# wolfecameron/GIST

Hardware: AMD Instinct MI355X
Metric: epochs/sec (higher is better)
Workload: dtype f32 (projection products from 3 bf16 pieces per operand = all 24 bits, 6 cross terms, fp32 accumulation)

## Files before the change

### gist_amd/csrc/gemm_b3.hip

```cpp
#include <stdlib.h>
#include <string.h>

#include <type_traits>

#include "common.h"

namespace gist {

typedef __bf16 bf16x8 __attribute__((ext_vector_type(8)));
typedef float b3_f32x4 __attribute__((ext_vector_type(4)));

constexpr int B3_TM = 256, B3_TN = 128, B3_BK = 32;
constexpr int B3_THREADS = 512;
constexpr int B3_STAGES = 2;
constexpr int B3_SKEW = 16;
constexpr int B3_KT_BYTES = B3_BK * 6;
constexpr int B3_A_BYTES = B3_TM * B3_KT_BYTES;
constexpr int B3_B_BYTES = B3_TN * B3_KT_BYTES;
constexpr int B3_BUF_BYTES = B3_A_BYTES + B3_B_BYTES;

__device__ __forceinline__ uint32_t b3_pack(__bf16 lo, __bf16 hi) {
    return (uint32_t)__builtin_bit_cast(unsigned short, lo) |
           ((uint32_t)__builtin_bit_cast(unsigned short, hi) << 16);
}

__device__ __forceinline__ void b3_emit(const float (&v)[8], uint16_t *__restrict__ dst) {
    uint32_t w[3][4];
#pragma unroll
    for (int j = 0; j < 4; ++j) {
        __bf16 p[2][3];
#pragma unroll
        for (int h = 0; h < 2; ++h) {
            const float x = v[2 * j + h];
            p[h][0] = (__bf16)x;
            const float r1 = x - (float)p[h][0];
            p[h][1] = (__bf16)r1;
            const float r2 = r1 - (float)p[h][1];
            p[h][2] = (__bf16)r2;
        }
#pragma unroll
        for (int q = 0; q < 3; ++q) w[q][j] = b3_pack(p[0][q], p[1][q]);
    }
#pragma unroll
    for (int q = 0; q < 3; ++q)
        *reinterpret_cast<uint4 *>(dst + 8 * q) = make_uint4(w[q][0], w[q][1], w[q][2], w[q][3]);
}

__global__ __launch_bounds__(256) void b3_dual_split_kernel(B3Dual d, int64_t ldd_r, int64_t ldd_t,
                                                            float keep) {
    __shared__ float tile[64][65];
    const int c0 = blockIdx.x * 64, r0 = blockIdx.y * 64;
    const int t = threadIdx.x;
    const int c4 = (t & 15) * 4;
    const uint64_t sm = d.seed * 0x9E3779B97F4A7C15ULL;
    const float inv24 = 1.0f / 16777216.0f;
#pragma unroll
    for (int i = 0; i < 4; ++i) {
        const int rr = (t >> 4) + 16 * i;
        const int64_t r = r0 + rr;
        float v[4] = {0.f, 0.f, 0.f, 0.f};
        if (r < d.rows) {
            const float *p = d.src + r * d.ld + c0 + c4;
            if (c0 + c4 + 3 < d.cols && d.vec4) {
                const float4 q = *reinterpret_cast<const float4 *>(p);
                v[0] = q.x; v[1] = q.y; v[2] = q.z; v[3] = q.w;
            } else {
#pragma unroll
                for (int j = 0; j < 4; ++j)
                    if (c0 + c4 + j < d.cols) v[j] = p[j];
            }
            if (d.p > 0.f) {
                const uint64_t idx0 = d.offset + (uint64_t)r * (uint64_t)d.cols + (uint64_t)(c0 + c4);
#pragma unroll
                for (int j = 0; j < 4; ++j) {
                    const uint64_t idx = idx0 + j;
                    const uint64_t h = splitmix64((idx >> 1) + sm);
                    const uint32_t w = (idx & 1) ? (uint32_t)(h >> 32) : (uint32_t)h;
                    v[j] *= ((float)(w >> 8) * inv24 >= d.p) ? keep : 0.f;
                }
            }
        }
        tile[rr][c4 + 0] = v[0]; tile[rr][c4 + 1] = v[1];
        tile[rr][c4 + 2] = v[2]; tile[rr][c4 + 3] = v[3];
    }
    __syncthreads();
    if (d.col_partials != nullptr && t < 64 && c0 + t < d.cols && r0 < d.rows) {
        float s0 = 0.f, s1 = 0.f, s2 = 0.f, s3 = 0.f;
#pragma unroll
        for (int r = 0; r < 64; r += 4) {
            s0 += tile[r][t]; s1 += tile[r + 1][t]; s2 += tile[r + 2][t]; s3 += tile[r + 3][t];
        }
        d.col_partials[(int64_t)blockIdx.y * d.cols + c0 + t] = (s0 + s1) + (s2 + s3);
    }
    const int kb = t & 7;
#pragma unroll
    for (int i = 0; i < 2; ++i) {
        const int q = (t >> 3) + 32 * i;
        if (d.dst_r != nullptr && r0 + q < d.rows && c0 + kb * 8 < ldd_r) {
            float v[8];
#pragma unroll
            for (int j = 0; j < 8; ++j) v[j] = tile[q][kb * 8 + j];
            b3_emit(v, d.dst_r + ((int64_t)(r0 + q) * ldd_r + c0 + kb * 8) * 3);
        }
        if (d.dst_t != nullptr && c0 + q < d.cols && r0 + kb * 8 < ldd_t) {
            float v[8];
#pragma unroll
            for (int j = 0; j < 8; ++j) v[j] = tile[kb * 8 + j][q];
            b3_emit(v, d.dst_t + ((int64_t)(c0 + q) * ldd_t + r0 + kb * 8) * 3);
        }
    }
}

struct B3Args {
    const uint16_t *a; int64_t lda;
    const uint16_t *b; int64_t ldb;
    const float *bias;
    float *c; int64_t ldc;
    int m, n, kpad;
    int tiles_m, tiles_n;
    int kt_per_split;
    int64_t split_stride;
    int dp_tiles, tail_splits, tail_kt;
    float *tail_partials;
};

template <int NI>
__device__ __forceinline__ void b3_dma_offsets(int64_t ld, int rows, int row0, int first, int lane,
                                                uint32_t (&off)[NI]) {
#pragma unroll
    for (int jj = 0; jj < NI; ++jj) {
        const int inst = first + jj;
        const int slot = (inst % 3) * 64 + lane;
        const int rs = slot / 12;
        const int chunk = (slot % 12) ^ ((rs >> 3) << 1);
        const int r = (inst / 3) * 16 + rs;
        const int dr = min(r, rows - 1 - row0);
        off[jj] = (uint32_t)((int64_t)dr * ld * 6 + chunk * 16);
    }
}

__device__ __forceinline__ void b3_mfma(b3_f32x4 &acc, const bf16x8 &a, const bf16x8 &b) {
    asm volatile("v_mfma_f32_16x16x32_bf16 %0, %1, %2, %0" : "+v"(acc) : "v"(a), "v"(b));
}

template <int NI>
__device__ __forceinline__ void b3_dma_image(const char *base, const uint32_t (&off)[NI], char *image,
                                             int first) {
    __amdgpu_buffer_rsrc_t rsrc = __builtin_amdgcn_make_buffer_rsrc(
        const_cast<char *>(base), 0, 0x7fffffff, 0x00020000);
#pragma unroll
    for (int jj = 0; jj < NI; ++jj)
        __builtin_amdgcn_raw_ptr_buffer_load_lds(
            rsrc, (__attribute__((address_space(3))) void *)(image + (first + jj) * 1024), 16, off[jj],
            0, 0, 0);
}

__global__ __launch_bounds__(B3_THREADS, 2) void gemm_b3_kernel(B3Args g) {
    extern __shared__ __attribute__((aligned(16))) char b3_smem[];
    constexpr int NI = 4, NJ = 4;
    const int nwg = g.dp_tiles;
    const int orig = blockIdx.x;
    const bool tail = orig >= nwg;
    const int tail_tile = tail ? (orig - nwg) / g.tail_splits : 0;
    const int tail_slice = tail ? (orig - nwg) % g.tail_splits : 0;
    const int qd = nwg / kXcds, rm = nwg % kXcds, xcd = orig % kXcds;
    const int L = tail ? nwg + tail_tile
                       : (xcd < rm ? xcd * (qd + 1) : rm * (qd + 1) + (xcd - rm) * qd) + orig / kXcds;
    constexpr int GM = 8;
    const int width = GM * g.tiles_n;
    const int group = L / width;
    const int first_m = group * GM;
    const int gsz = min(g.tiles_m - first_m, GM);
    const int bm = first_m + (L % width) % gsz;
    const int bn = (L % width) / gsz;
    const int row0 = bm * B3_TM, col0 = bn * B3_TN;
    const int kt0 = tail ? tail_slice * g.tail_kt : (int)blockIdx.y * g.kt_per_split;
    const int n_kt = min(g.kpad / B3_BK - kt0, tail ? g.tail_kt : g.kt_per_split);

    const int lane = threadIdx.x & 63;
    const int wave = __builtin_amdgcn_readfirstlane(threadIdx.x >> 6);
    const int wm = wave >> 1, wn = wave & 1;
    const int rr = lane & 15, kg = lane >> 4;

    b3_f32x4 acc[NI][NJ];
#pragma unroll
    for (int i = 0; i < NI; ++i)
#pragma unroll
        for (int j = 0; j < NJ; ++j)
#pragma unroll
            for (int e = 0; e < 4; ++e) acc[i][j][e] = 0.f;

    constexpr int NWAVES = B3_THREADS / 64;
    constexpr int DA = B3_TM / 16 * 3 / NWAVES, DB = B3_TN / 16 * 3 / NWAVES;
    uint32_t offA[DA], offB[DB];
    b3_dma_offsets<DA>(g.lda, g.m, row0, DA * wave, lane, offA);
    b3_dma_offsets<DB>(g.ldb, g.n, col0, DB * wave, lane, offB);
    const char *originA = reinterpret_cast<const char *>(g.a) + (int64_t)row0 * g.lda * 6 + (int64_t)kt0 * B3_KT_BYTES;
    const char *originB = reinterpret_cast<const char *>(g.b) + (int64_t)col0 * g.ldb * 6 + (int64_t)kt0 * B3_KT_BYTES;
    auto dma = [&](int buf, int kt) {
        char *sa = b3_smem + buf * B3_BUF_BYTES;
        b3_dma_image<DA>(originA + (int64_t)kt * B3_KT_BYTES, offA, sa, DA * wave);
        b3_dma_image<DB>(originB + (int64_t)kt * B3_KT_BYTES, offB, sa + B3_A_BYTES, DB * wave);
    };

    const char *fa[B3_STAGES][3], *fb[B3_STAGES][3];
#pragma unroll
    for (int p = 0; p < 3; ++p) {
        const int c = 3 * kg + p;
        const int in_slab = (rr * 12 + (c ^ ((rr >> 3) << 1))) * 16;
#pragma unroll
        for (int st = 0; st < B3_STAGES; ++st) {
            fa[st][p] = b3_smem + st * B3_BUF_BYTES + wm * NI * 3072 + in_slab;
            fb[st][p] = b3_smem + st * B3_BUF_BYTES + B3_A_BYTES + wn * NJ * 3072 + in_slab;
        }
    }

    const bool live = __builtin_amdgcn_readfirstlane(row0 + wm * (16 * NI) < g.m);
    bf16x8 a[NI][3], b[NJ][3];
    auto read_head = [&](auto st_c) {
        constexpr int st = decltype(st_c)::value;
        if (!live) return;
#pragma unroll
        for (int j = 0; j < NJ; ++j) b[j][0] = *reinterpret_cast<const bf16x8 *>(fb[st][0] + j * 3072);
#pragma unroll
        for (int i = 0; i < NI; ++i) a[i][1] = *reinterpret_cast<const bf16x8 *>(fa[st][1] + i * 3072);
#pragma unroll
        for (int i = 0; i < NI; ++i) a[i][2] = *reinterpret_cast<const bf16x8 *>(fa[st][2] + i * 3072);
    };
    auto read_rest = [&](auto st_c) {
        constexpr int st = decltype(st_c)::value;
        if (!live) return;
#pragma unroll
        for (int j = 0; j < NJ; ++j) b[j][1] = *reinterpret_cast<const bf16x8 *>(fb[st][1] + j * 3072);
#pragma unroll
        for (int i = 0; i < NI; ++i) a[i][0] = *reinterpret_cast<const bf16x8 *>(fa[st][0] + i * 3072);
#pragma unroll
        for (int j = 0; j < NJ; ++j) b[j][2] = *reinterpret_cast<const bf16x8 *>(fb[st][2] + j * 3072);
    };
    constexpr int pa[6] = {1, 2, 1, 0, 0, 0};
    constexpr int pb[6] = {0, 0, 1, 0, 1, 2};
    constexpr int B3_MID = 4 * NI * NJ;

    dma(0, 0);
    __builtin_amdgcn_s_waitcnt(0x0f70);
    __syncthreads();
    dma(1, 1);
    read_head(std::integral_constant<int, 0>{});

    auto mfmas = [&](auto t0_c, auto t1_c) {
        constexpr int t0 = decltype(t0_c)::value, t1 = decltype(t1_c)::value;
        if (!live) return;
#pragma unroll
        for (int t = t0; t < t1; ++t) {
            const int term = t / (NI * NJ), i = (t % (NI * NJ)) / NJ, j = t % NJ;
            b3_mfma(acc[i][j], a[i][pa[term]], b[j][pb[term]]);
        }
    };
    const int last_kt = n_kt - 1;
    auto kstep = [&](auto cur_c, auto late_c, int kt) {
        constexpr int cur = decltype(cur_c)::value;
        constexpr int skew = decltype(late_c)::value * B3_SKEW;
        using I = std::integral_constant<int, 0>;
        __builtin_amdgcn_sched_barrier(0);
        __builtin_amdgcn_s_setprio(1);
        mfmas(I{}, std::integral_constant<int, skew>{});
        __builtin_amdgcn_sched_barrier(0);
        read_rest(cur_c);
        __builtin_amdgcn_sched_barrier(0);
        mfmas(std::integral_constant<int, skew>{}, std::integral_constant<int, B3_MID>{});
        __builtin_amdgcn_sched_barrier(0);
        __builtin_amdgcn_s_waitcnt(0x0070);
        __syncthreads();
        mfmas(std::integral_constant<int, B3_MID>{}, std::integral_constant<int, B3_MID + skew>{});
        __builtin_amdgcn_sched_barrier(0);
        dma(cur, min(kt + 2, last_kt));
        read_head(std::integral_constant<int, cur ^ 1>{});
        __builtin_amdgcn_sched_barrier(0);
        mfmas(std::integral_constant<int, B3_MID + skew>{}, std::integral_constant<int, 6 * NI * NJ>{});
        __builtin_amdgcn_s_setprio(0);
        __builtin_amdgcn_sched_barrier(0);
    };
    auto run = [&](auto late_c) {
        using C0 = std::integral_constant<int, 0>;
        using C1 = std::integral_constant<int, 1>;
        for (int kt = 0; kt < n_kt; kt += 2) {
            kstep(C0{}, late_c, kt);
            kstep(C1{}, late_c, kt + 1);
        }
    };
    if (wave >= 4) run(std::integral_constant<int, 1>{});
    else run(std::integral_constant<int, 0>{});
    __builtin_amdgcn_s_waitcnt(0x0070);

    asm volatile("s_nop 15\n\ts_nop 15" ::: "memory");
    const int rows_valid = min(g.m - row0, B3_TM);
    if (tail) {
        const bool rows_live = wm * (16 * NI) < rows_valid;
        b3_f32x4 *mine = reinterpret_cast<b3_f32x4 *>(g.tail_partials) +
                         (int64_t)(tail_tile * g.tail_splits + tail_slice) * (NI * NJ * B3_THREADS) + threadIdx.x;
        if (rows_live) {
#pragma unroll
            for (int i = 0; i < NI; ++i)
#pragma unroll
                for (int j = 0; j < NJ; ++j) mine[(i * NJ + j) * B3_THREADS] = acc[i][j];
        }
        return;
    }
    float *cbase = g.c + (int64_t)blockIdx.y * g.split_stride + (int64_t)row0 * g.ldc + col0;
    __amdgpu_buffer_rsrc_t crsrc = __builtin_amdgcn_make_buffer_rsrc(
        cbase, 0, (int)((int64_t)rows_valid * g.ldc * 4), 0x00020000);
    const uint32_t ldc_b = (uint32_t)g.ldc * 4;
    uint32_t cvoff[NJ];
    float bv[NJ];
#pragma unroll
    for (int j = 0; j < NJ; ++j) {
        const int cl = wn * (16 * NJ) + j * 16 + rr;
        const bool ok = col0 + cl < g.n;
        cvoff[j] = ok ? (uint32_t)(wm * (16 * NI) + 4 * kg) * ldc_b + (uint32_t)cl * 4 : 0x7fffffffu;
        bv[j] = (g.bias != nullptr && ok) ? g.bias[col0 + cl] : 0.f;
    }
#pragma unroll
    for (int i = 0; i < NI; ++i)
#pragma unroll
        for (int e = 0; e < 4; ++e) {
            const uint32_t roff = (uint32_t)(i * 16 + e) * ldc_b;
#pragma unroll
            for (int j = 0; j < NJ; ++j) {
                const float v = acc[i][j][e] + bv[j];
                if (rows_valid == B3_TM)
                    __builtin_amdgcn_raw_buffer_store_b32(__float_as_uint(v), crsrc, cvoff[j], roff, 0);
                else
                    __builtin_amdgcn_raw_buffer_store_b32(__float_as_uint(v), crsrc, cvoff[j] + roff, 0, 0);
            }
        }
}

constexpr int B3W_TN = 256;
constexpr int B3W_B_BYTES = B3W_TN * B3_KT_BYTES;
constexpr int B3W_LDS_BYTES = B3_A_BYTES + 2 * B3W_B_BYTES;

__global__ __launch_bounds__(B3_THREADS, 1) void gemm_b3_wide_kernel(B3Args g) {
    extern __shared__ __attribute__((aligned(16))) char b3_smem[];
    constexpr int NI = 4, NJ = 8;
    const int nwg = g.dp_tiles;
    const int orig = blockIdx.x;
    const int qd = nwg / kXcds, rm = nwg % kXcds, xcd = orig % kXcds;
    const int L = (xcd < rm ? xcd * (qd + 1) : rm * (qd + 1) + (xcd - rm) * qd) + orig / kXcds;
    constexpr int GM = 8;
    const int width = GM * g.tiles_n;
    const int group = L / width;
    const int first_m = group * GM;
    const int gsz = min(g.tiles_m - first_m, GM);
    const int bm = first_m + (L % width) % gsz;
    const int bn = (L % width) / gsz;
    const int row0 = bm * B3_TM, col0 = bn * B3W_TN;
    const int n_kt = g.kpad / B3_BK;

    const int lane = threadIdx.x & 63;
    const int wave = __builtin_amdgcn_readfirstlane(threadIdx.x >> 6);
    const int wm = wave >> 1, wn = wave & 1;
    const int rr = lane & 15, kg = lane >> 4;

    b3_f32x4 acc[NI][NJ];
#pragma unroll
    for (int i = 0; i < NI; ++i)
#pragma unroll
        for (int j = 0; j < NJ; ++j)
#pragma unroll
            for (int e = 0; e < 4; ++e) acc[i][j][e] = 0.f;

    constexpr int NWAVES = B3_THREADS / 64;
    constexpr int DA = B3_TM / 16 * 3 / NWAVES, DB = B3W_TN / 16 * 3 / NWAVES;
    uint32_t offA[DA], offB[DB];
    b3_dma_offsets<DA>(g.lda, g.m, row0, DA * wave, lane, offA);
    b3_dma_offsets<DB>(g.ldb, g.n, col0, DB * wave, lane, offB);
    const char *originA = reinterpret_cast<const char *>(g.a) + (int64_t)row0 * g.lda * 6;
    const char *originB = reinterpret_cast<const char *>(g.b) + (int64_t)col0 * g.ldb * 6;
    auto dma = [&](int bbuf, int kt) {
        b3_dma_image<DA>(originA + (int64_t)kt * B3_KT_BYTES, offA, b3_smem, DA * wave);
        b3_dma_image<DB>(originB + (int64_t)kt * B3_KT_BYTES, offB, b3_smem + B3_A_BYTES + bbuf * B3W_B_BYTES,
                         DB * wave);
    };

    const char *fa[3], *fb[2][3];
#pragma unroll
    for (int p = 0; p < 3; ++p) {
        const int c = 3 * kg + p;
        const int in_slab = (rr * 12 + (c ^ ((rr >> 3) << 1))) * 16;
        fa[p] = b3_smem + wm * NI * 3072 + in_slab;
#pragma unroll
        for (int st = 0; st < 2; ++st) fb[st][p] = b3_smem + B3_A_BYTES + st * B3W_B_BYTES + wn * NJ * 3072 + in_slab;
    }

    auto body = [&](auto live_c) {
        constexpr bool live = decltype(live_c)::value;
        bf16x8 a[NI][3], b[2][3];
        auto read_a = [&](auto p_c) {
            constexpr int p = decltype(p_c)::value;
            if constexpr (!live) return;
#pragma unroll
            for (int i = 0; i < NI; ++i) a[i][p] = *reinterpret_cast<const bf16x8 *>(fa[p] + i * 3072);
        };
        auto read_b = [&](auto st_c, auto pair_c, auto p_c) {
            constexpr int st = decltype(st_c)::value, pair = decltype(pair_c)::value, p = decltype(p_c)::value;
            if constexpr (!live) return;
#pragma unroll
            for (int jj = 0; jj < 2; ++jj) b[jj][p] = *reinterpret_cast<const bf16x8 *>(fb[st][p] + (2 * pair + jj) * 3072);
        };
        constexpr int pa[6] = {1, 2, 1, 0, 0, 0};
        constexpr int pb[6] = {0, 0, 1, 0, 1, 2};
        auto mfmas = [&](auto pair_c, auto t0_c, auto t1_c) {
            constexpr int pair = decltype(pair_c)::value, t0 = decltype(t0_c)::value, t1 = decltype(t1_c)::value;
            if constexpr (!live) return;
#pragma unroll
            for (int term = t0; term < t1; ++term)
#pragma unroll
                for (int jj = 0; jj < 2; ++jj)
#pragma unroll
                    for (int i = 0; i < NI; ++i) b3_mfma(acc[i][2 * pair + jj], a[i][pa[term]], b[jj][pb[term]]);
        };
        using I0 = std::integral_constant<int, 0>;
        using I1 = std::integral_constant<int, 1>;
        using I2 = std::integral_constant<int, 2>;
        using I3 = std::integral_constant<int, 3>;

        dma(0, 0);
        __builtin_amdgcn_s_waitcnt(0x0f70);
        __syncthreads();
        read_a(I1{}); read_a(I2{});
        read_b(I0{}, I0{}, I0{}); read_b(I0{}, I0{}, I1{}); read_b(I0{}, I0{}, I2{});
        read_a(I0{});
        __builtin_amdgcn_s_waitcnt(0xc07f);

        const int last_kt = n_kt - 1;
        auto kstep = [&](auto cur_c, int kt) {
            constexpr int cur = decltype(cur_c)::value;
            auto pair_block = [&](auto pair_c) {
                constexpr int pair = decltype(pair_c)::value;
                using S = std::integral_constant<int, pair < 3 ? cur : (cur ^ 1)>;
                using P = std::integral_constant<int, pair < 3 ? pair + 1 : 0>;
                __builtin_amdgcn_sched_barrier(0);
                mfmas(pair_c, I0{}, I3{});
                __builtin_amdgcn_sched_barrier(0);
                if constexpr (pair == 0) {
                    __builtin_amdgcn_s_waitcnt(0xc07f);
                    __syncthreads();
                    dma(cur ^ 1, min(kt + 1, last_kt));
                }
                if constexpr (pair == 3) {
                    __builtin_amdgcn_s_waitcnt(0x0070);
                    __syncthreads();
                    read_a(I1{}); read_a(I2{});
                }
                __builtin_amdgcn_sched_barrier(0);
                mfmas(pair_c, I3{}, std::integral_constant<int, 4>{});
                __builtin_amdgcn_sched_barrier(0);
                read_b(S{}, P{}, I0{});
                __builtin_amdgcn_sched_barrier(0);
                mfmas(pair_c, std::integral_constant<int, 4>{}, std::integral_constant<int, 5>{});
                if constexpr (pair == 3) __builtin_amdgcn_s_waitcnt(0xc27f);
                __builtin_amdgcn_sched_barrier(0);
                read_b(S{}, P{}, I1{});
                __builtin_amdgcn_sched_barrier(0);
                mfmas(pair_c, std::integral_constant<int, 5>{}, std::integral_constant<int, 6>{});
                __builtin_amdgcn_sched_barrier(0);
                read_b(S{}, P{}, I2{});
                if constexpr (pair == 3) read_a(I0{});
            };
            __builtin_amdgcn_s_setprio(1);
            pair_block(I0{});
            pair_block(I1{});
            pair_block(I2{});
            pair_block(I3{});
            __builtin_amdgcn_s_setprio(0);
            __builtin_amdgcn_sched_barrier(0);
        };
        for (int kt = 0; kt < n_kt; kt += 2) {
            kstep(I0{}, kt);
            kstep(I1{}, kt + 1);
        }
    };
    if (__builtin_amdgcn_readfirstlane(row0 + wm * (16 * NI) < g.m)) body(std::true_type{});
    else body(std::false_type{});
    __builtin_amdgcn_s_waitcnt(0x0070);

    asm volatile("s_nop 15\n\ts_nop 15" ::: "memory");
    const int rows_valid = min(g.m - row0, B3_TM);
    float *cbase = g.c + (int64_t)row0 * g.ldc + col0;
    __amdgpu_buffer_rsrc_t crsrc = __builtin_amdgcn_make_buffer_rsrc(
        cbase, 0, (int)((int64_t)rows_valid * g.ldc * 4), 0x00020000);
    const uint32_t ldc_b = (uint32_t)g.ldc * 4;
    uint32_t cvoff[NJ];
    float bv[NJ];
#pragma unroll
    for (int j = 0; j < NJ; ++j) {
        const int cl = wn * (16 * NJ) + j * 16 + rr;
        const bool ok = col0 + cl < g.n;
        cvoff[j] = ok ? (uint32_t)(wm * (16 * NI) + 4 * kg) * ldc_b + (uint32_t)cl * 4 : 0x7fffffffu;
        bv[j] = (g.bias != nullptr && ok) ? g.bias[col0 + cl] : 0.f;
    }
#pragma unroll
    for (int i = 0; i < NI; ++i)
#pragma unroll
        for (int e = 0; e < 4; ++e) {
            const uint32_t roff = (uint32_t)(i * 16 + e) * ldc_b;
#pragma unroll
            for (int j = 0; j < NJ; ++j) {
                const float v = acc[i][j][e] + bv[j];
                if (rows_valid == B3_TM)
                    __builtin_amdgcn_raw_buffer_store_b32(__float_as_uint(v), crsrc, cvoff[j], roff, 0);
                else
                    __builtin_amdgcn_raw_buffer_store_b32(__float_as_uint(v), crsrc, cvoff[j] + roff, 0, 0);
            }
        }
}

__global__ __launch_bounds__(B3_THREADS) void gemm_b3_tail_sum_kernel(B3Args g) {
    constexpr int NI = 4, NJ = 4, GM = 8;
    const int L = g.dp_tiles + (int)blockIdx.x;
    const int width = GM * g.tiles_n;
    const int first_m = (L / width) * GM;
    const int gsz = min(g.tiles_m - first_m, GM);
    const int row0 = (first_m + (L % width) % gsz) * B3_TM, col0 = ((L % width) / gsz) * B3_TN;
    const int lane = threadIdx.x & 63, wave = threadIdx.x >> 6;
    const int wm = wave >> 1, wn = wave & 1, rr = lane & 15, kg = lane >> 4;
    const int reg = blockIdx.y, i = reg / NJ, j = reg % NJ;
    const int row = row0 + wm * (16 * NI) + i * 16 + 4 * kg, col = col0 + wn * (16 * NJ) + j * 16 + rr;
    if (row0 + wm * (16 * NI) >= g.m || col >= g.n) return;
    const b3_f32x4 *part = reinterpret_cast<const b3_f32x4 *>(g.tail_partials) +
                           ((int64_t)blockIdx.x * g.tail_splits * (NI * NJ) + reg) * B3_THREADS + threadIdx.x;
    b3_f32x4 sum = part[0];
    for (int q = 1; q < g.tail_splits; ++q) sum += part[(int64_t)q * (NI * NJ) * B3_THREADS];
    const float bv = g.bias != nullptr ? g.bias[col] : 0.f;
#pragma unroll
    for (int e = 0; e < 4; ++e)
        if (row + e < g.m) g.c[(int64_t)(row + e) * g.ldc + col] = sum[e] + bv;
}

int64_t b3_kpad(int64_t k) { return ceil_div(k, 2 * B3_BK) * (2 * B3_BK); }

int b3_splits(int64_t m, int64_t n, int64_t k) {
    const int64_t tiles = ceil_div(m, B3_TM) * ceil_div(n, B3_TN);
    const int64_t n_kt = b3_kpad(k) / B3_BK;
    const int forced = (int)tune(GIST_TUNE_GEMM_SPLITS);
    int64_t s = forced > 0 ? forced : (tiles >= 192 ? 1 : 256 / tiles);
    if (forced <= 0 && tiles > 128 && tiles < 192) {
        int64_t best = n_kt + 4;
        for (int64_t c = 2; c <= 4; ++c) {
            const int64_t per = ceil_div(ceil_div(n_kt, c), 2) * 2;
            const int64_t cost = ceil_div(tiles * c, 256) * per + 8;
            if (per >= 8 && cost < best) { best = cost; s = c; }
        }
    }
    if (forced <= 0 && s > n_kt / 8) s = n_kt / 8;
    if (s > n_kt / 2) s = n_kt / 2;
    if (s < 1) s = 1;
    const int64_t per = ceil_div(ceil_div(n_kt, s), 2) * 2;
    return (int)ceil_div(n_kt, per);
}
struct B3Tail { int dp_tiles, splits, kt; };
constexpr int B3_CUS = 256;
static B3Tail b3_tail(int64_t m, int64_t n, int64_t k) {
    const int64_t tiles = ceil_div(m, B3_TM) * ceil_div(n, B3_TN);
    B3Tail t{(int)tiles, 1, 0};
    if (tune(GIST_TUNE_B3_TAIL) == 1.0 || tiles <= B3_CUS) return t;
    const int64_t r = tiles % B3_CUS;
    if (r == 0 || r > B3_CUS / 2) return t;
    const int64_t n_kt = b3_kpad(k) / B3_BK;
    int64_t s = B3_CUS / r;
    if (s > n_kt / 8) s = n_kt / 8;
    if (s < 2) return t;
    const int64_t per = ceil_div(ceil_div(n_kt, s), 2) * 2;
    s = ceil_div(n_kt, per);
    if (s < 2) return t;
    t.dp_tiles = (int)(tiles - r); t.splits = (int)s; t.kt = (int)per;
    return t;
}
static int64_t b3_tail_bytes(int64_t m, int64_t n, int64_t k) {
    const B3Tail t = b3_tail(m, n, k);
    if (t.splits < 2) return 0;
    const int64_t r = ceil_div(m, B3_TM) * ceil_div(n, B3_TN) - t.dp_tiles;
    return r * t.splits * (int64_t)(B3_TM * B3_TN * 4);
}
static bool b3_wide(int64_t m, int64_t n, int64_t k) {
    if (tune(GIST_TUNE_B3_WIDE) == 1.0) return false;
    if (ceil_div(m, B3_TM) * ceil_div(n, B3W_TN) < B3_CUS) return false;
    return b3_splits(m, n, k) == 1 && b3_tail(m, n, k).splits < 2;
}
int64_t b3_slab_bytes(int64_t m, int64_t n, int64_t k) {
    const int s = b3_splits(m, n, k);
    return s > 1 ? (int64_t)s * m * n * 4 : b3_tail_bytes(m, n, k);
}

static bool b3_shape_ok(int64_t m, int64_t n, int64_t k, double default_min_gflop) {
    const double t_gflop = tune(GIST_TUNE_H3_MIN_GFLOP), t_tiles = tune(GIST_TUNE_H3_MIN_TILES);
    const double min_gflop = t_gflop > 0.0 ? t_gflop : default_min_gflop;
    const int min_wgs = t_tiles > 0.0 ? (int)t_tiles : 128;
    if (t_tiles <= 0.0 && (m < 64 || n < 64 || k < 64)) return false;
    if (m < 1 || n < 1 || k < 1) return false;
    const int64_t tiles = ceil_div(m, B3_TM) * ceil_div(n, B3_TN);
    if (tiles * b3_splits(m, n, k) < min_wgs) return false;
    if (t_tiles <= 0.0 && (double)m * (double)n < 0.6 * (double)(tiles * B3_TM * B3_TN)) return false;
    if (2.0 * (double)m * (double)n * (double)k < min_gflop * 1e9) return false;
    if (b3_kpad(k) * 6 >= (1LL << 23)) return false;
    return true;
}
bool b3_eligible(int64_t m, int64_t n, int64_t k) { return h3_mode() == 2 && b3_shape_ok(m, n, k, 16.0); }
bool b3_eligible_kept(int64_t m, int64_t n, int64_t k) { return b3_shape_ok(m, n, k, 9.0); }

static int64_t b3_operand_bytes(int64_t m, int64_t n, int64_t k) {
    return ceil_div((m + n) * b3_kpad(k) * 6 + 512, 256) * 256;
}
int64_t b3_workspace_bytes(int64_t m, int64_t n, int64_t k) {
    if (!b3_eligible(m, n, k)) return 0;
    return b3_operand_bytes(m, n, k) + b3_slab_bytes(m, n, k);
}

int b3_dual_split(const B3Dual &d, hipStream_t st) {
    if (d.rows <= 0 || d.cols <= 0) return GIST_OK;
    const int64_t ldd_r = b3_kpad(d.cols), ldd_t = b3_kpad(d.rows);
    const int64_t gx = ceil_div(d.dst_r ? ldd_r : d.cols, 64), gy = ceil_div(d.dst_t ? ldd_t : d.rows, 64);
    B3Dual dd = d;
    dd.vec4 = aligned16(d.src) && d.ld % 4 == 0;
    hipLaunchKernelGGL(b3_dual_split_kernel, dim3((unsigned)gx, (unsigned)gy), dim3(256), 0, st, dd, ldd_r,
                       ldd_t, d.p > 0.f ? 1.0f / (1.0f - d.p) : 1.0f);
    return launch_status("b3_dual_split");
}

int b3_gemm_presplit(const char *name, const uint16_t *sa, const uint16_t *sb, const float *bias, float *c,
                     int64_t ldc, int64_t m, int64_t n, int64_t k, float *slabs, int64_t slab_bytes,
                     hipStream_t st, int *deferred) {
    static DeviceOnce once;
    int dev;
    if (once.needed(&dev)) {
        hipError_t e = hipFuncSetAttribute(reinterpret_cast<const void *>(&gemm_b3_kernel),
                                           hipFuncAttributeMaxDynamicSharedMemorySize, B3_STAGES * B3_BUF_BYTES);
        if (e == hipSuccess)
            e = hipFuncSetAttribute(reinterpret_cast<const void *>(&gemm_b3_wide_kernel),
                                    hipFuncAttributeMaxDynamicSharedMemorySize, B3W_LDS_BYTES);
        if (e != hipSuccess) {
            set_error("%s: hipFuncSetAttribute: %s", name, hipGetErrorString(e));
            return GIST_ELAUNCH;
        }
        once.done(dev);
    }
    if (ldc * B3_TM * 4 >= (1LL << 31)) {
        set_error("%s: leading dimension of the output >= 2^21 elements on the bf16x3 path", name);
        return GIST_EINVAL;
    }
    B3Args g;
    const int64_t kpad = b3_kpad(k);
    g.a = sa; g.lda = kpad; g.b = sb; g.ldb = kpad; g.bias = bias; g.c = c; g.ldc = ldc;
    g.m = (int)m; g.n = (int)n; g.kpad = (int)kpad;
    g.tiles_m = (int)ceil_div(m, B3_TM);
    g.tiles_n = (int)ceil_div(n, B3_TN);
    const int64_t n_kt = kpad / B3_BK;
    int splits = b3_splits(m, n, k);
    if (splits > 1 && (slabs == nullptr || slab_bytes < (int64_t)splits * m * n * 4)) splits = 1;
    g.kt_per_split = (int)(ceil_div(ceil_div(n_kt, splits), 2) * 2);
    splits = (int)ceil_div(n_kt, g.kt_per_split);
    g.split_stride = 0;
    if (splits > 1) { g.c = slabs; g.ldc = n; g.split_stride = m * n; g.bias = nullptr; }
    g.dp_tiles = g.tiles_m * g.tiles_n; g.tail_splits = 1; g.tail_kt = 0;
    g.tail_partials = nullptr;
    unsigned grid_x = (unsigned)g.dp_tiles;
    if (splits == 1 && slabs != nullptr && aligned16(slabs)) {
        const B3Tail t = b3_tail(m, n, k);
        if (t.splits > 1 && slab_bytes >= b3_tail_bytes(m, n, k)) {
            const int r = g.dp_tiles - t.dp_tiles;
            g.dp_tiles = t.dp_tiles; g.tail_splits = t.splits; g.tail_kt = t.kt;
            g.tail_partials = slabs;
            grid_x = (unsigned)(t.dp_tiles + r * t.splits);
        }
    }
    const int64_t slot = timer_begin(tl_timer, 2, m, n, k, st);
    if (b3_wide(m, n, k) && splits == 1 && g.tail_splits == 1) {
        g.tiles_n = (int)ceil_div(n, B3W_TN);
        g.dp_tiles = g.tiles_m * g.tiles_n;
        hipLaunchKernelGGL(gemm_b3_wide_kernel, dim3((unsigned)g.dp_tiles), dim3(B3_THREADS), B3W_LDS_BYTES, st, g);
        const int rc = launch_status(name);
        if (deferred) *deferred = 1;
        timer_end(tl_timer, slot, st);
        return rc;
    }
    hipLaunchKernelGGL(gemm_b3_kernel, dim3(grid_x, (unsigned)splits),
                       dim3(B3_THREADS), B3_STAGES * B3_BUF_BYTES, st, g);
    int rc = launch_status(name);
    if (rc == GIST_OK && g.tail_splits > 1) {
        hipLaunchKernelGGL(gemm_b3_tail_sum_kernel, dim3((grid_x - (unsigned)g.dp_tiles) / (unsigned)g.tail_splits, 16),
                           dim3(B3_THREADS), 0, st, g);
        rc = launch_status(name);
    }
    if (deferred) *deferred = splits;
    else if (rc == GIST_OK && splits > 1) rc = splitk_reduce(name, slabs, m * n, splits, bias, c, ldc, m, n, st);
    timer_end(tl_timer, slot, st);
    return rc;
}

int b3_gemm(const char *name, bool a_kc, bool b_kc, const float *a, int64_t lda, const float *b,
            int64_t ldb, const float *bias, float *c, int64_t ldc, int64_t m, int64_t n, int64_t k,
            void *ws, int64_t ws_bytes, hipStream_t st) {
    if (!b3_eligible(m, n, k)) return 0;
    if (ldc * B3_TM * 4 >= (1LL << 31)) return 0;
    if (ws == nullptr || !aligned16(ws) || ws_bytes < b3_workspace_bytes(m, n, k)) return 0;
    const int64_t kpad = b3_kpad(k);
    uint16_t *sa = static_cast<uint16_t *>(ws);
    uint16_t *sb = sa + m * kpad * 3;
    float *slabs = reinterpret_cast<float *>(static_cast<char *>(ws) + b3_operand_bytes(m, n, k));
    auto split = [&](bool kc, const float *src, int64_t ld, int64_t rows, uint16_t *dst) {
        B3Dual d{};
        d.src = src; d.ld = ld;
        if (kc) { d.rows = rows; d.cols = k; d.dst_r = dst; }
        else { d.rows = k; d.cols = rows; d.dst_t = dst; }
        return b3_dual_split(d, st);
    };
    int rc = split(a_kc, a, lda, m, sa);
    if (rc != GIST_OK) return rc;
    rc = split(b_kc, b, ldb, n, sb);
    if (rc != GIST_OK) return rc;
    rc = b3_gemm_presplit(name, sa, sb, bias, c, ldc, m, n, k, slabs, b3_slab_bytes(m, n, k), st, nullptr);
    return rc == GIST_OK ? 1 : rc;
}

}
```

Before: 5.177.

## Extend wide bf16x3 GEMM kernel to split-K and stream-K tails with a cost-model planner

The 256x256 wide kernel now handles split-K (through blockIdx.y and an offset K range) and tail-split tiles, whose partial accumulators go to a slab and are summed by a templated tail-sum kernel. A new planner estimates wave-quantised cost for the narrow and wide tilings, weighting each wide k-step at 1.85 narrow steps, and picks the cheaper one. Before, the wide kernel was used only when no split or tail was needed. The goal is better per-tile reuse on shapes that need splitting. The risk is that the cost heuristic picks the wide path where its lower occupancy or extra partial traffic costs more than it saves.

```diff
diff --git a/gist_amd/csrc/gemm_b3.hip b/gist_amd/csrc/gemm_b3.hip
--- a/gist_amd/csrc/gemm_b3.hip
+++ b/gist_amd/csrc/gemm_b3.hip
@@ -344,8 +344,12 @@
     constexpr int NI = 4, NJ = 8;
     const int nwg = g.dp_tiles;
     const int orig = blockIdx.x;
+    const bool tail = orig >= nwg;
+    const int tail_tile = tail ? (orig - nwg) / g.tail_splits : 0;
+    const int tail_slice = tail ? (orig - nwg) % g.tail_splits : 0;
     const int qd = nwg / kXcds, rm = nwg % kXcds, xcd = orig % kXcds;
-    const int L = (xcd < rm ? xcd * (qd + 1) : rm * (qd + 1) + (xcd - rm) * qd) + orig / kXcds;
+    const int L = tail ? nwg + tail_tile
+                       : (xcd < rm ? xcd * (qd + 1) : rm * (qd + 1) + (xcd - rm) * qd) + orig / kXcds;
     constexpr int GM = 8;
     const int width = GM * g.tiles_n;
     const int group = L / width;
@@ -354,7 +358,8 @@
     const int bm = first_m + (L % width) % gsz;
     const int bn = (L % width) / gsz;
     const int row0 = bm * B3_TM, col0 = bn * B3W_TN;
-    const int n_kt = g.kpad / B3_BK;
+    const int kt0 = tail ? tail_slice * g.tail_kt : (int)blockIdx.y * g.kt_per_split;
+    const int n_kt = min(g.kpad / B3_BK - kt0, tail ? g.tail_kt : g.kt_per_split);
 
     const int lane = threadIdx.x & 63;
     const int wave = __builtin_amdgcn_readfirstlane(threadIdx.x >> 6);
@@ -374,8 +379,8 @@
     uint32_t offA[DA], offB[DB];
     b3_dma_offsets<DA>(g.lda, g.m, row0, DA * wave, lane, offA);
     b3_dma_offsets<DB>(g.ldb, g.n, col0, DB * wave, lane, offB);
-    const char *originA = reinterpret_cast<const char *>(g.a) + (int64_t)row0 * g.lda * 6;
-    const char *originB = reinterpret_cast<const char *>(g.b) + (int64_t)col0 * g.ldb * 6;
+    const char *originA = reinterpret_cast<const char *>(g.a) + (int64_t)row0 * g.lda * 6 + (int64_t)kt0 * B3_KT_BYTES;
+    const char *originB = reinterpret_cast<const char *>(g.b) + (int64_t)col0 * g.ldb * 6 + (int64_t)kt0 * B3_KT_BYTES;
     auto dma = [&](int bbuf, int kt) {
         b3_dma_image<DA>(originA + (int64_t)kt * B3_KT_BYTES, offA, b3_smem, DA * wave);
         b3_dma_image<DB>(originB + (int64_t)kt * B3_KT_BYTES, offB, b3_smem + B3_A_BYTES + bbuf * B3W_B_BYTES,
@@ -486,7 +491,19 @@
 
     asm volatile("s_nop 15\n\ts_nop 15" ::: "memory");
     const int rows_valid = min(g.m - row0, B3_TM);
-    float *cbase = g.c + (int64_t)row0 * g.ldc + col0;
+    if (tail) {
+        const bool rows_live = wm * (16 * NI) < rows_valid;
+        b3_f32x4 *mine = reinterpret_cast<b3_f32x4 *>(g.tail_partials) +
+                         (int64_t)(tail_tile * g.tail_splits + tail_slice) * (NI * NJ * B3_THREADS) + threadIdx.x;
+        if (rows_live) {
+#pragma unroll
+            for (int i = 0; i < NI; ++i)
+#pragma unroll
+                for (int j = 0; j < NJ; ++j) mine[(i * NJ + j) * B3_THREADS] = acc[i][j];
+        }
+        return;
+    }
+    float *cbase = g.c + (int64_t)blockIdx.y * g.split_stride + (int64_t)row0 * g.ldc + col0;
     __amdgpu_buffer_rsrc_t crsrc = __builtin_amdgcn_make_buffer_rsrc(
         cbase, 0, (int)((int64_t)rows_valid * g.ldc * 4), 0x00020000);
     const uint32_t ldc_b = (uint32_t)g.ldc * 4;
@@ -515,13 +532,14 @@
         }
 }
 
+template <int NJ>
 __global__ __launch_bounds__(B3_THREADS) void gemm_b3_tail_sum_kernel(B3Args g) {
-    constexpr int NI = 4, NJ = 4, GM = 8;
+    constexpr int NI = 4, GM = 8, TN = 32 * NJ;
     const int L = g.dp_tiles + (int)blockIdx.x;
     const int width = GM * g.tiles_n;
     const int first_m = (L / width) * GM;
     const int gsz = min(g.tiles_m - first_m, GM);
-    const int row0 = (first_m + (L % width) % gsz) * B3_TM, col0 = ((L % width) / gsz) * B3_TN;
+    const int row0 = (first_m + (L % width) % gsz) * B3_TM, col0 = ((L % width) / gsz) * TN;
     const int lane = threadIdx.x & 63, wave = threadIdx.x >> 6;
     const int wm = wave >> 1, wn = wave & 1, rr = lane & 15, kg = lane >> 4;
     const int reg = blockIdx.y, i = reg / NJ, j = reg % NJ;
@@ -560,8 +578,7 @@
 }
 struct B3Tail { int dp_tiles, splits, kt; };
 constexpr int B3_CUS = 256;
-static B3Tail b3_tail(int64_t m, int64_t n, int64_t k) {
-    const int64_t tiles = ceil_div(m, B3_TM) * ceil_div(n, B3_TN);
+static B3Tail b3_tail(int64_t tiles, int64_t k) {
     B3Tail t{(int)tiles, 1, 0};
     if (tune(GIST_TUNE_B3_TAIL) == 1.0 || tiles <= B3_CUS) return t;
     const int64_t r = tiles % B3_CUS;
@@ -576,21 +593,42 @@
     t.dp_tiles = (int)(tiles - r); t.splits = (int)s; t.kt = (int)per;
     return t;
 }
-static int64_t b3_tail_bytes(int64_t m, int64_t n, int64_t k) {
-    const B3Tail t = b3_tail(m, n, k);
-    if (t.splits < 2) return 0;
-    const int64_t r = ceil_div(m, B3_TM) * ceil_div(n, B3_TN) - t.dp_tiles;
-    return r * t.splits * (int64_t)(B3_TM * B3_TN * 4);
-}
-static bool b3_wide(int64_t m, int64_t n, int64_t k) {
-    if (tune(GIST_TUNE_B3_WIDE) == 1.0) return false;
-    if (ceil_div(m, B3_TM) * ceil_div(n, B3W_TN) < B3_CUS) return false;
-    return b3_splits(m, n, k) == 1 && b3_tail(m, n, k).splits < 2;
-}
-int64_t b3_slab_bytes(int64_t m, int64_t n, int64_t k) {
-    const int s = b3_splits(m, n, k);
-    return s > 1 ? (int64_t)s * m * n * 4 : b3_tail_bytes(m, n, k);
-}
+
+struct B3Plan { bool wide; int splits; B3Tail tail; };
+constexpr double B3W_KT = 1.85;
+
+static int64_t b3_tiles(int64_t m, int64_t n, bool wide) {
+    return ceil_div(m, B3_TM) * ceil_div(n, wide ? B3W_TN : B3_TN);
+}
+static double b3_cost(int64_t tiles, int64_t n_kt, int s, const B3Tail &t, double kt_cost) {
+    if (s > 1) {
+        const int64_t per = ceil_div(ceil_div(n_kt, s), 2) * 2;
+        return (double)(ceil_div(tiles * s, B3_CUS) * per) * kt_cost + 4.0;
+    }
+    if (t.splits > 1) return (double)(t.dp_tiles / B3_CUS * n_kt + t.kt) * kt_cost + 4.0;
+    return (double)(ceil_div(tiles, B3_CUS) * n_kt) * kt_cost;
+}
+static B3Plan b3_plan(int64_t m, int64_t n, int64_t k) {
+    const int64_t n_kt = b3_kpad(k) / B3_BK;
+    B3Plan nar{false, b3_splits(m, n, k), B3Tail{}};
+    const int64_t tn = b3_tiles(m, n, false);
+    nar.tail = nar.splits == 1 ? b3_tail(tn, k) : B3Tail{(int)tn, 1, 0};
+    const int mode = (int)tune(GIST_TUNE_B3_WIDE);
+    if (mode == 1) return nar;
+    const int64_t tw = b3_tiles(m, n, true);
+    const B3Plan wid{true, nar.splits, nar.splits == 1 ? b3_tail(tw, k) : B3Tail{(int)tw, 1, 0}};
+    const double wcost = b3_cost(tw, n_kt, wid.splits, wid.tail, B3W_KT);
+    if (mode == 2) return wid;
+    const double ncost = b3_cost(tn, n_kt, nar.splits, nar.tail, 1.0);
+    return wcost < ncost ? wid : nar;
+}
+static int64_t b3_plan_bytes(const B3Plan &p, int64_t m, int64_t n) {
+    if (p.splits > 1) return (int64_t)p.splits * m * n * 4;
+    if (p.tail.splits < 2) return 0;
+    const int64_t r = b3_tiles(m, n, p.wide) - p.tail.dp_tiles;
+    return r * p.tail.splits * (int64_t)(B3_TM * (p.wide ? B3W_TN : B3_TN) * 4);
+}
+int64_t b3_slab_bytes(int64_t m, int64_t n, int64_t k) { return b3_plan_bytes(b3_plan(m, n, k), m, n); }
 
 static bool b3_shape_ok(int64_t m, int64_t n, int64_t k, double default_min_gflop) {
     const double t_gflop = tune(GIST_TUNE_H3_MIN_GFLOP), t_tiles = tune(GIST_TUNE_H3_MIN_TILES);
@@ -652,43 +690,36 @@
     const int64_t kpad = b3_kpad(k);
     g.a = sa; g.lda = kpad; g.b = sb; g.ldb = kpad; g.bias = bias; g.c = c; g.ldc = ldc;
     g.m = (int)m; g.n = (int)n; g.kpad = (int)kpad;
+    const int64_t n_kt = kpad / B3_BK;
+    B3Plan pl = b3_plan(m, n, k);
+    const int64_t need = b3_plan_bytes(pl, m, n);
+    if (need > 0 && (slabs == nullptr || slab_bytes < need || (pl.splits == 1 && !aligned16(slabs)))) {
+        const int64_t tiles = b3_tiles(m, n, false);
+        pl = B3Plan{false, 1, b3_tail(tiles, k)};
+        if (slabs == nullptr || !aligned16(slabs) || slab_bytes < b3_plan_bytes(pl, m, n)) pl.tail = B3Tail{(int)tiles, 1, 0};
+    }
     g.tiles_m = (int)ceil_div(m, B3_TM);
-    g.tiles_n = (int)ceil_div(n, B3_TN);
-    const int64_t n_kt = kpad / B3_BK;
-    int splits = b3_splits(m, n, k);
-    if (splits > 1 && (slabs == nullptr || slab_bytes < (int64_t)splits * m * n * 4)) splits = 1;
-    g.kt_per_split = (int)(ceil_div(ceil_div(n_kt, splits), 2) * 2);
-    splits = (int)ceil_div(n_kt, g.kt_per_split);
+    g.tiles_n = (int)ceil_div(n, pl.wide ? B3W_TN : B3_TN);
+    g.kt_per_split = (int)(ceil_div(ceil_div(n_kt, pl.splits), 2) * 2);
+    const int splits = (int)ceil_div(n_kt, g.kt_per_split);
     g.split_stride = 0;
     if (splits > 1) { g.c = slabs; g.ldc = n; g.split_stride = m * n; g.bias = nullptr; }
-    g.dp_tiles = g.tiles_m * g.tiles_n; g.tail_splits = 1; g.tail_kt = 0;
-    g.tail_partials = nullptr;
-    unsigned grid_x = (unsigned)g.dp_tiles;
-    if (splits == 1 && slabs != nullptr && aligned16(slabs)) {
-        const B3Tail t = b3_tail(m, n, k);
-        if (t.splits > 1 && slab_bytes >= b3_tail_bytes(m, n, k)) {
-            const int r = g.dp_tiles - t.dp_tiles;
-            g.dp_tiles = t.dp_tiles; g.tail_splits = t.splits; g.tail_kt = t.kt;
-            g.tail_partials = slabs;
-            grid_x = (unsigned)(t.dp_tiles + r * t.splits);
-        }
-    }
+    g.dp_tiles = pl.tail.dp_tiles; g.tail_splits = pl.tail.splits; g.tail_kt = pl.tail.kt;
+    g.tail_partials = pl.tail.splits > 1 ? slabs : nullptr;
+    const int tail_tiles = g.tiles_m * g.tiles_n - g.dp_tiles;
+    const unsigned grid_x = (unsigned)(g.dp_tiles + tail_tiles * g.tail_splits);
     const int64_t slot = timer_begin(tl_timer, 2, m, n, k, st);
-    if (b3_wide(m, n, k) && splits == 1 && g.tail_splits == 1) {
-        g.tiles_n = (int)ceil_div(n, B3W_TN);
-        g.dp_tiles = g.tiles_m * g.tiles_n;
-        hipLaunchKernelGGL(gemm_b3_wide_kernel, dim3((unsigned)g.dp_tiles), dim3(B3_THREADS), B3W_LDS_BYTES, st, g);
-        const int rc = launch_status(name);
-        if (deferred) *deferred = 1;
-        timer_end(tl_timer, slot, st);
-        return rc;
-    }
-    hipLaunchKernelGGL(gemm_b3_kernel, dim3(grid_x, (unsigned)splits),
-                       dim3(B3_THREADS), B3_STAGES * B3_BUF_BYTES, st, g);
+    if (pl.wide)
+        hipLaunchKernelGGL(gemm_b3_wide_kernel, dim3(grid_x, (unsigned)splits), dim3(B3_THREADS), B3W_LDS_BYTES, st, g);
+    else
+        hipLaunchKernelGGL(gemm_b3_kernel, dim3(grid_x, (unsigned)splits), dim3(B3_THREADS), B3_STAGES * B3_BUF_BYTES,
+                           st, g);
     int rc = launch_status(name);
     if (rc == GIST_OK && g.tail_splits > 1) {
-        hipLaunchKernelGGL(gemm_b3_tail_sum_kernel, dim3((grid_x - (unsigned)g.dp_tiles) / (unsigned)g.tail_splits, 16),
-                           dim3(B3_THREADS), 0, st, g);
+        if (pl.wide)
+            hipLaunchKernelGGL(gemm_b3_tail_sum_kernel<8>, dim3((unsigned)tail_tiles, 32), dim3(B3_THREADS), 0, st, g);
+        else
+            hipLaunchKernelGGL(gemm_b3_tail_sum_kernel<4>, dim3((unsigned)tail_tiles, 16), dim3(B3_THREADS), 0, st, g);
         rc = launch_status(name);
     }
     if (deferred) *deferred = splits;
```

Result: no change. 5.209, median of 6 (+0.6%).
